# Basant1861/MPC-MMD

Measured on AMD Instinct MI355X. Metric: MPC optimizer steps/s (batch=1024,H=30,obs_samp=500) @1/2/4/8 GPU; % HBM roofline, higher is better.
Workload: dtype f32; 1 GPU; static obs, mmd_opt, batch=1024 rollouts, H=30, num_obs=10, obs_samples=484 (n=22, M=n^2); cost=mmd_opt, global_batch=1024, num_batch=1024, num_prime=30, num_obs=10, num_reduced=22, noise=gaussian, parallelism=config-sharded x1

## Files before the change

### mpc-mmd_amd/csrc/betacem_select.hpp

```cpp
#pragma once
#include "betacem_common.hpp"

namespace mpcmmd {

namespace {

template <int NQ, class V>
DEVI void load_keys(V val, int M, uint32_t* key) {
  const int lane = tidx() & 63;
#pragma unroll
  for (int q = 0; q < NQ; ++q) {
    const int j = lane + 64 * q;
    const float v = val(min(j, M - 1));
    key[q] = j < M ? sort_key_abs(v) : 0u;
  }
}

template <int NQ, int NB>
DEVI void find_thresholds(const uint32_t (*key)[NQ], int nb, int n, uint32_t* T, bool* exact) {
  constexpr int NP = (NB + 1) / 2;
#pragma unroll
  for (int u = 0; u < NB; ++u) {
    T[u] = 0x80000000u;
    exact[u] = u >= nb;
  }
  for (int bit = 30; bit >= 0; --bit) {
    int packed[NP];
#pragma unroll
    for (int i = 0; i < NP; ++i) packed[i] = 0;
#pragma unroll
    for (int u = 0; u < NB; ++u) {
      if (exact[u]) continue;
      const uint32_t cand = T[u] | (1u << bit);
      int c = 0;
#pragma unroll
      for (int q = 0; q < NQ; ++q) c += key[u][q] >= cand;
      packed[u >> 1] += c << (16 * (u & 1));
    }
    bool all = true;
#pragma unroll
    for (int i = 0; i < NP; ++i) {
      const int tot = wave_total(packed[i]);
#pragma unroll
      for (int h = 0; h < 2; ++h) {
        const int u = 2 * i + h;
        if (u >= NB || exact[u]) continue;
        const int cnt = (tot >> (16 * h)) & 0xFFFF;
        if (cnt >= n) T[u] |= 1u << bit;
        exact[u] = cnt == n;
        all = all && exact[u];
      }
    }
    if (all) break;
  }
}

template <int NQ>
DEVI void emit_top(const uint32_t* key, uint32_t T, bool exact, int n, int32_t* out, int* scratch) {
  const int lane = tidx() & 63;
  int need = 0;
  unsigned long long eqm[NQ];
  if (!exact) {
    int gt = 0;
#pragma unroll
    for (int q = 0; q < NQ; ++q) gt += __popcll(__ballot(key[q] > T));
    need = n - gt;
#pragma unroll
    for (int q = 0; q < NQ; ++q) eqm[q] = __ballot(key[q] == T);
  } else {
#pragma unroll
    for (int q = 0; q < NQ; ++q) eqm[q] = 0ull;
  }
  const unsigned long long above = lane == 63 ? 0ull : (~0ull << (lane + 1));
  int* lj = scratch;
  uint32_t* lk = reinterpret_cast<uint32_t*>(scratch + 64);
  int base = 0;
  int later_eq = 0;
#pragma unroll
  for (int q = 0; q < NQ; ++q) later_eq += __popcll(eqm[q]);
#pragma unroll
  for (int q = 0; q < NQ; ++q) {
    later_eq -= __popcll(eqm[q]);
    const int larger = later_eq + __popcll(eqm[q] & above);
    const bool sel = exact ? key[q] >= T : (key[q] > T || (key[q] == T && larger < need));
    const unsigned long long sm = __ballot(sel);
    if (sel) {
      const int pos = base + __popcll(sm & ((1ull << lane) - 1ull));
      lj[pos] = lane + 64 * q;
      lk[pos] = key[q];
    }
    base += __popcll(sm);
  }
  wave_sync();
  const int j = lane < n ? lj[lane] : 0;
  const uint32_t k = lane < n ? lk[lane] : 0xFFFFFFFFu;
  int r = 0;
  for (int c = 0; c < n; ++c) {
    const uint32_t kc = __builtin_amdgcn_readlane(k, c);
    r += (kc < k) || (kc == k && c < lane);
  }
  if (lane < n) out[r] = j;
  wave_sync();
}

template <int NQ, int R>
DEVI bool emit_window(const uint32_t* key, uint32_t T, int n, int32_t* out, unsigned long long* cand) {
  constexpr int cap = 64 * R;
  const int lane = tidx() & 63;
  const unsigned long long below = (1ull << lane) - 1ull;
  int c = 0;
#pragma unroll
  for (int q = 0; q < NQ; ++q) {
    const bool sel = key[q] >= T;
    const unsigned long long m = __ballot(sel);
    const int pos = c + __popcll(m & below);
    cand[sel && pos < cap ? pos : cap + 3] = (static_cast<unsigned long long>(key[q]) << 32) | uint32_t(lane + 64 * q);
    c += __popcll(m);
  }
  if (c > cap) return false;
  if (lane < 8) cand[c + lane] = 0ull;
  wave_sync();
  unsigned long long mine[R];
  int rank[R];
#pragma unroll
  for (int r = 0; r < R; ++r) {
    mine[r] = cand[lane + 64 * r];
    rank[r] = 0;
  }
  const ulonglong2* c2 = reinterpret_cast<const ulonglong2*>(cand);
  for (int e = 0; e < c; e += 8) {
    ulonglong2 v[4];
#pragma unroll
    for (int u = 0; u < 4; ++u) v[u] = c2[(e >> 1) + u];
#pragma unroll
    for (int u = 0; u < 4; ++u)
#pragma unroll
      for (int r = 0; r < R; ++r) rank[r] += int(v[u].x > mine[r]) + int(v[u].y > mine[r]);
  }
#pragma unroll
  for (int r = 0; r < R; ++r)
    if (lane + 64 * r < c && rank[r] < n) out[n - 1 - rank[r]] = int32_t(uint32_t(mine[r]));
  wave_sync();
  return true;
}

template <int CTRL, int ROWS = 0xF>
DEVI uint32_t dpp_umin_src(uint32_t v) {
  return uint32_t(__builtin_amdgcn_update_dpp(-1, int(v), CTRL, ROWS, 0xF, false));
}
DEVI uint32_t wave_min_u32(uint32_t v) {
  v = min(v, dpp_umin_src<0xB1>(v));
  v = min(v, dpp_umin_src<0x4E>(v));
  v = min(v, dpp_umin_src<0x124>(v));
  v = min(v, dpp_umin_src<0x128>(v));
  v = min(v, dpp_umin_src<0x142, 0xA>(v));
  v = min(v, dpp_umin_src<0x143, 0xC>(v));
  return uint32_t(__builtin_amdgcn_readlane(int(v), 63));
}

template <int NQ, int G>
DEVI uint32_t group_max_threshold(const uint32_t* key, int n, uint32_t* lm) {
  const int lane = tidx() & 63;
  uint32_t m = key[0];
#pragma unroll
  for (int q = 1; q < NQ; ++q) m = max(m, key[q]);
  if constexpr (G == 32) m = max(m, uint32_t(__builtin_amdgcn_update_dpp(0, int(m), 0xB1, 0xF, 0xF, false)));
  if (lane % (64 / G) == 0) lm[lane / (64 / G)] = m;
  wave_sync();
  int gt = 0;
  const uint4* l4 = reinterpret_cast<const uint4*>(lm);
#pragma unroll
  for (int e = 0; e < G / 4; ++e) {
    const uint4 v = l4[e];
    gt += int(v.x > m) + int(v.y > m) + int(v.z > m) + int(v.w > m);
  }
  const uint32_t t = wave_min_u32(gt < n ? m : 0xFFFFFFFFu);
  wave_sync();
  return t;
}

template <int NQ, int R, int G, class Row, class Out>
DEVI void select_walk(Row row, Out out, int first, int last, int stride, int M, int n, unsigned long long* cand,
                      uint32_t* lm, int* scratch) {
  uint32_t key[NQ], nxt[NQ];
  load_keys<NQ>(row(first), M, key);
  for (int s = first; s < last; s += stride) {
    load_keys<NQ>(row(min(s + stride, last - 1)), M, nxt);
    bool done = false;
    if (M <= 64 * R)
      done = emit_window<NQ, R>(key, 0x80000000u, n, out(s), cand);
    else if (G > 0 && n <= G * 3 / 4)
      done = emit_window<NQ, R>(key, group_max_threshold<NQ, (G > 0 ? G : 64)>(key, n, lm), n, out(s), cand);
    if (!done) {
      uint32_t Tn[1];
      bool ex[1];
      find_thresholds<NQ, 1>(&key, 1, n, Tn, ex);
      emit_top<NQ>(key, Tn[0], ex[0], n, out(s), scratch);
    }
#pragma unroll
    for (int q = 0; q < NQ; ++q) key[q] = nxt[q];
  }
}

template <int NQ, int R, int G>
DEVI void bselect_wave(const Params& p, int tb, int b, int g, int W, unsigned long long* cand, uint32_t* lm,
                       int* scratch) {
  const int M = p.M, M1 = M + 1, n = p.n;
  int32_t* sel = p.bsel + size_t(b) * kBetaSamples * n;
  float* sig = p.bsig + size_t(b) * kBetaSamples;
  const float* E = p.belite + (size_t(tb & 1) * p.Bt + b) * kBetaElite * M1;
  const int ys = ygen_stride(M);
  const float* Y = p.ygen + size_t(b) * kBzCols * ys;
  const float* z0 = p.beta_z0;
  auto row = [&](int s) {
    const float* r = tb == 0 ? z0 + size_t(s) * M1 : (s < kBetaElite ? E + size_t(s) * M1 : Y + size_t(s - kBetaElite) * ys);
    const bool scale = tb == 0;
    return [=](int j) { return scale ? float(kSqrt20 * double(r[j])) : r[j]; };
  };
  const int s_lo = first_sample(tb);
  if (s_lo + g >= kBetaSamples) return;
  select_walk<NQ, R, G>(row, [&](int s) { return sel + s * n; }, s_lo + g, kBetaSamples, W, M, n, cand, lm, scratch);
  const int lane = tidx() & 63;
  for (int s = s_lo + g + lane * W; lane < 16 && s < kBetaSamples; s += 16 * W) {
    const float v = row(s)(M);
    sig[s] = tb == 0 ? fmaxf(v, 0.01f) : v;
  }
}

}

}
```

### mpc-mmd_amd/csrc/k_bcem_small.hip

```cpp
#define MPCMMD_OPAQUE_TIDX 1
#include "betacem_elite.hpp"
#include "betacem_kernel.hpp"
#include "betacem_qp.hpp"
#include "betacem_sample.hpp"
#include "betacem_select.hpp"

namespace mpcmmd {

namespace {

HDI size_t small_sel_bytes(int R) { return size_t(64 * R + 8) * 8 + 64 * 4 + 128 * 4; }
HDI size_t small_lds(int M, int n, int R, int W) {
  size_t b = size_t(W) * small_sel_bytes(R) + size_t(kNew) * ygen_stride(M) * 4;
  const size_t k = ker_lds(M, n, ker_scratch(M, n, 1, W)).total;
  const size_t d = dir_lds(M, n).total, e = elite_lds(M + 1, W).total;
  const size_t q = (size_t(kBetaSamples) * tri_stride(n) + kQpZeros) * 4;
  const size_t g = size_t(W) * 4 * 32 * 8;
  const size_t gl = ((gen_lds_bytes(M) + 15) & ~size_t(15)) + tblk_lds_bytes(M);
  b = b > q ? b : q;
  b = b > g ? b : g;
  b = b > gl ? b : gl;
  b = b > k ? b : k;
  b = b > d ? b : d;
  b = b > e ? b : e;
  return b;
}

HDI size_t small_persist_off(int M, int n, int R, int W) { return (small_lds(M, n, R, W) + 15) & ~size_t(15); }
HDI size_t small_persist_bytes(int M) { return size_t(M) * (kMomStride + kFeatStride) * 4; }

#define SMALL_STAMP(p, slot)                                                             \
  do {                                                                                   \
    if (tidx() == 0 && (p).dbgw)                                                    \
      (p).dbgw[size_t(32768 + blockIdx.x) * 8 + (slot)] = __builtin_amdgcn_s_memrealtime(); \
  } while (0)

template <int NQ, int R, int G, int NP, int NV4, int GNB, int W>
__global__ __launch_bounds__(64 * W) void k_bcem_small(Params p0, int persist) {
  constexpr int kSmallWaves = W, kSmallThreads = 64 * W;
  extern __shared__ __attribute__((aligned(16))) char smem[];
  const int cand = blockIdx.x;
  const int tid = tidx();
  const int w = __builtin_amdgcn_readfirstlane(tid >> 6);
  const float4* mom_l = nullptr;
  const float4* feat_l = nullptr;
  if (persist) {
    const int M = p0.M, b = p0.b0 + cand;
    float4* pm = reinterpret_cast<float4*>(smem + small_persist_off(M, p0.n, R, W));
    float4* pf = pm + M * (kMomStride / 4);
    const float4* gm = reinterpret_cast<const float4*>(p0.bmom + size_t(b) * M * kMomStride);
    const float4* gf = reinterpret_cast<const float4*>(p0.featr + size_t(b) * M * kFeatStride);
    for (int i = tid; i < M * (kMomStride / 4); i += kSmallThreads) pm[i] = gm[i];
    for (int i = tid; i < M * (kFeatStride / 4); i += kSmallThreads) pf[i] = gf[i];
    mom_l = pm;
    feat_l = pf;
    __syncthreads();
  }
  for (int tb = 0; tb < kBetaIters; ++tb) {
    typedef const Params __attribute__((address_space(4)))* KParams;
    KParams pk = (KParams)__builtin_amdgcn_kernarg_segment_ptr();
    asm volatile("" : "+s"(pk));
    const Params& p = *(const Params*)pk;
    const int b = p.b0 + cand, M = p.M, n = p.n;
    const int ntri = tri_stride(n);
    if (tb > 0) {
      if (tb == 5) SMALL_STAMP(p, 0);
      {
        const int Pp = pos_pad(M);
        const double2* gsrc = reinterpret_cast<const double2*>(p.gen + size_t(b) * Pp * kGenStride);
        const double2* msrc = reinterpret_cast<const double2*>(p.genm + size_t(b) * Pp);
        double2* dst = reinterpret_cast<double2*>(smem);
        const int ng = Pp * kGenRow, nm = Pp >> 1;
        for (int i = tid; i < ng + nm; i += kSmallThreads) dst[i] = i < ng ? gsrc[i] : msrc[i - ng];
        if (tid < 8) dst[ng + nm + tid] = double2{0.0, 0.0};
      }
      __syncthreads();
      {
        const double* lg = reinterpret_cast<const double*>(smem);
        double* Tl = reinterpret_cast<double*>(smem + ((gen_lds_bytes(M) + 15) & ~size_t(15)));
        bsample_tblocks(p, lg, Tl, w, kSmallWaves);
        __syncthreads();
        const int nblk = pos_pad(M) >> 4, units = kSampleTiles * ((nblk + sample_chunk(nblk) - 1) / sample_chunk(nblk));
        for (int u = w; u < units; u += kSmallWaves) bsample_unit_lds(p, tb, b, u % kSampleTiles, u / kSampleTiles, lg, Tl);
      }
      __syncthreads();
      if (tb == 5) SMALL_STAMP(p, 1);
      const int ys = ygen_stride(M);
      const float* Yl = reinterpret_cast<const float*>(smem + size_t(kSmallWaves) * small_sel_bytes(R));
      {
        const float4* src = reinterpret_cast<const float4*>(p.ygen + size_t(b) * kBzCols * ys);
        float4* dst = reinterpret_cast<float4*>(smem + size_t(kSmallWaves) * small_sel_bytes(R));
        for (int i = tid; i < kNew * (ys >> 2); i += kSmallThreads) dst[i] = src[i];
      }
      __syncthreads();
      char* sw = smem + size_t(w) * small_sel_bytes(R);
      unsigned long long* cand_l = reinterpret_cast<unsigned long long*>(sw);
      uint32_t* lm = reinterpret_cast<uint32_t*>(sw + size_t(64 * R + 8) * 8);
      int* scr = reinterpret_cast<int*>(sw + size_t(64 * R + 8) * 8 + 64 * 4);
      {
        int32_t* sel = p.bsel + size_t(b) * kBetaSamples * n;
        float* sig = p.bsig + size_t(b) * kBetaSamples;
        auto row = [&](int s) {
          const float* r = Yl + size_t(s - kBetaElite) * ys;
          return [=](int j) { return r[j]; };
        };
        const int s_lo = first_sample(tb), lane = tid & 63;
        if (s_lo + w < kBetaSamples) {
          select_walk<NQ, R, G>(row, [&](int s) { return sel + s * n; }, s_lo + w, kBetaSamples, kSmallWaves, M, n,
                                cand_l, lm, scr);
          for (int s2 = s_lo + w + lane * kSmallWaves; lane < 16 && s2 < kBetaSamples; s2 += 16 * kSmallWaves)
            sig[s2] = row(s2)(M);
        }
      }
    } else {
      for (int e = tid; e < kBetaSamples * n; e += kSmallThreads) p.bsel[size_t(b) * kBetaSamples * n + e] = p.sel0[e];
      for (int e = tid; e < kBetaSamples; e += kSmallThreads) p.bsig[size_t(b) * kBetaSamples + e] = p.sig0[e];
    }
    __syncthreads();
    if (tb == 5) SMALL_STAMP(p, 2);
    bkernel_body<kSmallWaves, false, true>(p, tb, cand, 0, 1, int(ker_scratch(M, n, tb, kSmallWaves)), smem, mom_l, feat_l);
    __syncthreads();
    if (tb == 5) SMALL_STAMP(p, 3);
    if (tb > 0) {
      const int total = bdirect_total(p, b, 1);
      if (total > 0) {
        bdirect_body<NV4, kSmallWaves>(p, tb, 1, 1, cand, 0, total, smem);
        __syncthreads();
      }
    }
    if (tb == 5) SMALL_STAMP(p, 4);
    {
      const int s_lo = first_sample(tb), per = kBetaSamples - s_lo;
      const float4* src = reinterpret_cast<const float4*>(p.bkred + (size_t(b) * kBetaSamples + s_lo) * ntri);
      float4* kl4 = reinterpret_cast<float4*>(smem);
      for (int i = tid; i < per * (ntri >> 2); i += kSmallThreads) kl4[i] = src[i];
      if (tid < kQpZeros) reinterpret_cast<float*>(smem)[per * ntri + tid] = 0.0f;
      __syncthreads();
      static_assert(kSmallThreads / 4 >= kBetaSamples, "one quad per QP");
      const int g = tid >> 2;
      const bool ok = g < per;
      const int gc = ok ? g : 0;
      bqp_solve<NP>(p, b, s_lo + gc, ok, reinterpret_cast<const float*>(smem) + size_t(gc) * ntri,
                    reinterpret_cast<const float*>(smem) + size_t(per) * ntri);
    }
    __syncthreads();
    if (tb == 5) SMALL_STAMP(p, 5);
    belite_body(p, tb, b, smem);
    __syncthreads();
    if (tb == 5) SMALL_STAMP(p, 6);
    {
      const int nblk = (M + 1 + 15) / 16;
      double* xl = reinterpret_cast<double*>(smem) + 32 * GNB * w;
      for (int blk = w; blk < nblk; blk += kSmallWaves * GNB) bgen_wave<GNB>(p, b, blk, kSmallWaves, xl);
    }
    __syncthreads();
    if (tb == 5) SMALL_STAMP(p, 7);
    if (tb == kBetaIters - 1 && p.bimin[b] >= kBetaElite) {
      bsigma_body(p, tb, b, reinterpret_cast<double*>(smem));
      __syncthreads();
    }
  }
}

}

constexpr int kSmallW512 = 8;
HDI int small_waves(int M) { return M <= 256 ? 16 : (M <= 512 ? kSmallW512 : 8); }

bool bcem_small_ok(const Params& p) {
  return p.gen_wave && p.M <= 256 && p.nb <= 512 && small_lds(p.M, p.n, 1, small_waves(p.M)) <= kLdsBudget;
}

void launch_bcem_small(const Params& p, hipStream_t s) {
  const int n = p.n, M = p.M, W = small_waves(M);
  const dim3 grid(p.nb), block(64 * W);
  const size_t lp = small_persist_off(M, n, 1, W) + small_persist_bytes(M);
  const int persist = lp <= kLdsBudget;
  const size_t lds = persist ? lp : small_lds(M, n, 1, W);
  if (M <= 64)
    hipLaunchKernelGGL((k_bcem_small<1, 1, 32, 8, 1, 1, 16>), grid, block, lds, s, p, persist);
  else if (M <= 128)
    hipLaunchKernelGGL((k_bcem_small<2, 1, 32, 12, 1, 1, 16>), grid, block, lds, s, p, persist);
  else if (M <= 256)
    hipLaunchKernelGGL((k_bcem_small<4, 1, 32, 16, 1, 1, 16>), grid, block, lds, s, p, persist);
  else if (M <= 512)
    hipLaunchKernelGGL((k_bcem_small<8, 1, 32, 24, 2, 16 / kSmallW512, kSmallW512>), grid, block, lds, s,
                       p, persist);
  else
    hipLaunchKernelGGL((k_bcem_small<12, 1, 32, 24, 3, 2, 8>), grid, block, lds, s, p, persist);
}

}
```

### mpc-mmd_amd/csrc/k_bsample.hip

```cpp
#include <algorithm>

#include "betacem_sample.hpp"
#include "betacem_select.hpp"

namespace mpcmmd {

namespace {

__global__ __launch_bounds__(256) void k_bsel0(Params p) {
  const int n = p.n, per = kBetaSamples * n + kBetaSamples;
  for (size_t x = size_t(blockIdx.x) * 256 + tidx(); x < size_t(p.nb) * per; x += size_t(gridDim.x) * 256) {
    const int c = int(x / per), e = int(x - size_t(c) * per), b = p.b0 + c;
    if (e < kBetaSamples * n)
      p.bsel[size_t(b) * kBetaSamples * n + e] = p.sel0[e];
    else
      p.bsig[size_t(b) * kBetaSamples + e - kBetaSamples * n] = p.sig0[e - kBetaSamples * n];
  }
}

template <int TPW>
__global__ __launch_bounds__(64 * sample_waves<TPW>()) void k_bsample(Params p, int tb) {
  const int b = p.b0 + blockIdx.x, M = p.M, Pp = pos_pad(M);
  const int lane = tidx() & 63, w = tidx() >> 6;
  const int r = lane & 15, h = lane >> 4;
  const int s0 = w * TPW * 16;
  MPCMMD_STAMP(p, 0);
  const double* G = p.gen + size_t(b) * Pp * kGenStride;
  const double* gm = p.genm + size_t(b) * Pp;
  const float* z = p.beta_z + size_t(tb - 1) * Pp * kBzCols;
  const int ys = ygen_stride(M);
  float* plane = p.ygen + size_t(b) * kBzCols * ys;
  d4 S[TPW], Sp[TPW], Ya[TPW], Yb[TPW];
#pragma unroll
  for (int t = 0; t < TPW; ++t) {
    S[t] = Sp[t] = d4{0.0, 0.0, 0.0, 0.0};
    Sp[t][2] = h == 3 ? 1.0 : 0.0;
  }
  const int nblk = Pp >> 4, cl = sample_chunk(nblk);
  const __amdgpu_buffer_rsrc_t yr = ygen_rsrc(plane, ys);
  const int vl = (2 * h * ys + r) * 4, v43 = h == 0 ? vl : kDropOffset;
  auto store = [&](const d4* Yv, int q0) {
    if (TPW == kSampleTiles && q0 + 15 < M)
      block_store_rows(Yv, yr, q0, ys, vl, v43);
    else
      block_store<TPW>(Yv, plane, q0, M, ys, s0, r, h);
  };
  SampleBlock<TPW> qa, qb;
  const SampleRsrc srs = sample_rsrc(G, gm, z, Pp, r, h);
  auto load = [&](SampleBlock<TPW>& q, int q0) {
    if constexpr (TPW == kSampleTiles)
      load_block_buf(q, srs, q0);
    else
      load_block(q, G, G + gen_uplane(Pp), gm, z, q0, s0, r, h);
  };
  load(qa, 0);
  for (int c = 0; c < nblk; c += 2) {
    const int p0 = c << 4;
    load(qb, p0 + 16);
    __builtin_amdgcn_sched_barrier(0);
    block_mfma(qa, S, Sp, Ya, r, h);
    __builtin_amdgcn_sched_barrier(0);
    if (c > 0) store(Yb, p0 - 16);
    __builtin_amdgcn_sched_barrier(0);
    load(qa, min(p0 + 32, Pp - 16));
    __builtin_amdgcn_sched_barrier(0);
    block_mfma(qb, S, Sp, Yb, r, h);
    if ((c + 2) % cl == 0)
#pragma unroll
      for (int t = 0; t < TPW; ++t) fold_chunk(Sp[t], S[t]);
    __builtin_amdgcn_sched_barrier(0);
    store(Ya, p0);
    __builtin_amdgcn_sched_barrier(0);
  }
  store(Yb, Pp - 16);
  MPCMMD_STAMP(p, 1);
}

__global__ __launch_bounds__(64 * kChunkWavesMax) void k_bsample_chunks(Params p, int tb) {
  __shared__ double dS[kChunkWavesMax - 1][3][64];
  const int b = p.b0 + blockIdx.x, M = p.M, Pp = pos_pad(M), nblk = Pp >> 4;
  const int lane = tidx() & 63, k = tidx() >> 6, P = blockDim.x >> 6;
  const int r = lane & 15, h = lane >> 4, s0 = blockIdx.y * 16;
  const int cl = sample_chunk(nblk), c0 = k * cl, c1 = min(nblk, c0 + cl);
  MPCMMD_STAMP(p, 0);
  const double* G = p.gen + size_t(b) * Pp * kGenStride;
  const double* gm = p.genm + size_t(b) * Pp;
  const float* z = p.beta_z + size_t(tb - 1) * Pp * kBzCols;
  const int ys = ygen_stride(M);
  float* plane = p.ygen + size_t(b) * kBzCols * ys;
  if (k < P - 1) {
    auto ld = [&](double (&wa)[4], double (&zz)[4], int c) {
#pragma unroll
      for (int kk = 0; kk < 4; ++kk) {
        const size_t pos = size_t(c) * 16 + 4 * kk + h;
        wa[kk] = G[pos * kGenRow + kGenW + r];
        zz[kk] = double(z[bz_index(int(pos), s0 + r)]);
      }
    };
    d4 Sl = d4{0.0, 0.0, 0.0, 0.0};
    double wa[4], zz[4], wn[4], zn[4];
    ld(wa, zz, c0);
    for (int c = c0; c < c1; ++c) {
      ld(wn, zn, min(c + 1, c1 - 1));
#pragma unroll
      for (int kk = 0; kk < 4; ++kk) Sl = mfma64(wa[kk], zz[kk], Sl);
#pragma unroll
      for (int kk = 0; kk < 4; ++kk) {
        wa[kk] = wn[kk];
        zz[kk] = zn[kk];
      }
    }
#pragma unroll
    for (int i = 0; i < 3; ++i) dS[k][i][lane] = Sl[i];
  }
  __syncthreads();
  d4 S[1] = {d4{0.0, 0.0, 0.0, 0.0}}, Sp[1] = {d4{0.0, 0.0, 0.0, 0.0}}, Ya[1], Yb[1];
  Sp[0][2] = h == 3 ? 1.0 : 0.0;
  for (int j = 0; j < k; ++j)
#pragma unroll
    for (int i = 0; i < 3; ++i) Sp[0][i] = Sp[0][i] + dS[j][i][lane];
  SampleBlock<1> qa, qb;
  const int pend = c1 << 4;
  load_block(qa, G, G + gen_uplane(Pp), gm, z, c0 << 4, s0, r, h);
  for (int c = c0; c < c1; c += 2) {
    const int p0 = c << 4;
    load_block(qb, G, G + gen_uplane(Pp), gm, z, p0 + 16, s0, r, h);
    __builtin_amdgcn_sched_barrier(0);
    block_mfma(qa, S, Sp, Ya, r, h);
    __builtin_amdgcn_sched_barrier(0);
    if (c > c0) block_store<1>(Yb, plane, p0 - 16, M, ys, s0, r, h);
    __builtin_amdgcn_sched_barrier(0);
    load_block(qa, G, G + gen_uplane(Pp), gm, z, min(p0 + 32, pend - 16), s0, r, h);
    __builtin_amdgcn_sched_barrier(0);
    block_mfma(qb, S, Sp, Yb, r, h);
    __builtin_amdgcn_sched_barrier(0);
    block_store<1>(Ya, plane, p0, M, ys, s0, r, h);
    __builtin_amdgcn_sched_barrier(0);
  }
  block_store<1>(Yb, plane, pend - 16, M, ys, s0, r, h);
  MPCMMD_STAMP(p, 1);
}

template <int NQ, int R, int G>
__global__ __launch_bounds__(64) void k_bselect(Params p, int tb) {
  __shared__ __attribute__((aligned(16))) unsigned long long cand[64 * R + 8];
  __shared__ __attribute__((aligned(16))) uint32_t lm[64];
  __shared__ int scratch[128];
  if (blockIdx.y == 0 && tidx() == 0) p.bdlcount[size_t(p.b0 + blockIdx.x) * kBetaIters + tb] = 0;
  bselect_wave<NQ, R, G>(p, tb, p.b0 + blockIdx.x, blockIdx.y, gridDim.y, cand, lm, scratch);
}

}

void launch_bsample(const Params& p, int tb, hipStream_t s) {
  if (p.nb >= 384) {
    hipLaunchKernelGGL((k_bsample<6>), dim3(p.nb), dim3(64 * sample_waves<6>()), 0, s, p, tb);
  } else {
    const int nblk = pos_pad(p.M) >> 4, cl = sample_chunk(nblk);
    hipLaunchKernelGGL(k_bsample_chunks, dim3(p.nb, kSampleTiles), dim3(64 * ((nblk + cl - 1) / cl)), 0, s, p, tb);
  }
}

void launch_bsel0(const Params& p, hipStream_t s) {
  const size_t total = size_t(p.nb) * (kBetaSamples * p.n + kBetaSamples);
  hipLaunchKernelGGL(k_bsel0, dim3(unsigned(std::min<size_t>((total + 255) / 256, 4096))), dim3(256), 0, s, p);
}

int sel_waves(int nb, int cap) { return std::max(4, std::min(nb <= 128 ? cap : 16, 16384 / std::max(1, nb))); }

template <int NQ>
void launch_bselect_q(const Params& p, int tb, hipStream_t s) {
  const dim3 grid(p.nb, sel_waves(p.nb, p.sel_cap));
  if (p.n <= 24)
    hipLaunchKernelGGL((k_bselect<NQ, 1, 32>), grid, dim3(64), 0, s, p, tb);
  else if (p.n <= 48)
    hipLaunchKernelGGL((k_bselect<NQ, 2, 64>), grid, dim3(64), 0, s, p, tb);
  else
    hipLaunchKernelGGL((k_bselect<NQ, 2, 0>), grid, dim3(64), 0, s, p, tb);
}

void launch_bselect(const Params& p, int tb, hipStream_t s) {
  const int nq = (p.M + 63) >> 6;
  switch (nq) {
#define MPCMMD_SEL_CASE(q) \
  case q:                  \
    return launch_bselect_q<q>(p, tb, s);
    MPCMMD_SEL_CASE(1)
    MPCMMD_SEL_CASE(2)
    MPCMMD_SEL_CASE(4)
    MPCMMD_SEL_CASE(8)
    MPCMMD_SEL_CASE(16)
#undef MPCMMD_SEL_CASE
    default:
      break;
  }
  if (nq <= 4) return launch_bselect_q<4>(p, tb, s);
  if (nq <= 8) return launch_bselect_q<8>(p, tb, s);
  if (nq <= 12) return launch_bselect_q<12>(p, tb, s);
  if (nq <= 16) return launch_bselect_q<16>(p, tb, s);
  if (nq <= 24) return launch_bselect_q<24>(p, tb, s);
  if (nq <= 32) return launch_bselect_q<32>(p, tb, s);
  if (nq <= 40) return launch_bselect_q<40>(p, tb, s);
  if (nq <= 48) return launch_bselect_q<48>(p, tb, s);
  return launch_bselect_q<64>(p, tb, s);
}

}
```

Measured before the change: 138.2 steps/s.

## Reuse previous top-n threshold and use 32-bit key window selection

Top-n selection now tries a 32-bit key window seeded with a threshold carried over from the previous sample of the same wave. It falls back to the group-max threshold, and then to the 64-bit window or the radix search when the window misses or ties collide. Keys are built with a saturating-add trick, row pointers are made wave-uniform, rows are indexed by byte offset, and the group-max count is split across lane pairs. The kernel also gets a minimum-waves launch bound to raise occupancy. The aim is to skip threshold computation and shrink shared-memory ranking traffic, at the cost of more branches and fallback paths.

```diff
diff --git a/mpc-mmd_amd/csrc/betacem_select.hpp b/mpc-mmd_amd/csrc/betacem_select.hpp
--- a/mpc-mmd_amd/csrc/betacem_select.hpp
+++ b/mpc-mmd_amd/csrc/betacem_select.hpp
@@ -5,15 +5,30 @@
 
 namespace {
 
+DEVI uint32_t select_key(float v) {
+  return __builtin_elementwise_add_sat(__float_as_uint(v) | 0x80000000u, 0x007FFFFEu);
+}
+
 template <int NQ, class V>
 DEVI void load_keys(V val, int M, uint32_t* key) {
-  const int lane = tidx() & 63;
-#pragma unroll
-  for (int q = 0; q < NQ; ++q) {
-    const int j = lane + 64 * q;
-    const float v = val(min(j, M - 1));
-    key[q] = j < M ? sort_key_abs(v) : 0u;
-  }
+  const uint32_t lane = tidx() & 63;
+#pragma unroll
+  for (int q = 0; q < NQ; ++q) {
+    const uint32_t j = lane + 64 * q;
+    const float v = val(4u * min(j, uint32_t(M - 1)));
+    key[q] = j < uint32_t(M) ? select_key(v) : 0u;
+  }
+}
+
+template <class T>
+DEVI T* scalar_ptr(T* p) {
+  const unsigned long long v = reinterpret_cast<unsigned long long>(p);
+  const uint32_t lo = __builtin_amdgcn_readfirstlane(uint32_t(v)), hi = __builtin_amdgcn_readfirstlane(uint32_t(v >> 32));
+  return reinterpret_cast<T*>((static_cast<unsigned long long>(hi) << 32) | lo);
+}
+
+DEVI float row_at(const float* r, uint32_t o) {
+  return *reinterpret_cast<const float*>(reinterpret_cast<const char*>(r) + o);
 }
 
 template <int NQ, int NB>
@@ -104,7 +119,7 @@
 }
 
 template <int NQ, int R>
-DEVI bool emit_window(const uint32_t* key, uint32_t T, int n, int32_t* out, unsigned long long* cand) {
+DEVI bool emit_window64(const uint32_t* key, uint32_t T, int n, int32_t* out, unsigned long long* cand) {
   constexpr int cap = 64 * R;
   const int lane = tidx() & 63;
   const unsigned long long below = (1ull << lane) - 1ull;
@@ -142,6 +157,76 @@
     if (lane + 64 * r < c && rank[r] < n) out[n - 1 - rank[r]] = int32_t(uint32_t(mine[r]));
   wave_sync();
   return true;
+}
+
+enum { kWinMiss = 0, kWinDone = 1, kWinTie = 2 };
+template <int NQ, int R>
+DEVI int emit_window32(const uint32_t* key, uint32_t T, int n, int KR, int32_t* out, uint32_t* ck, uint32_t* lm,
+                       uint32_t& Tc) {
+  constexpr int cap = 64 * R;
+  constexpr bool keep = NQ <= 16;
+  const int lane = tidx() & 63;
+  bool sel[keep ? NQ : 1];
+  unsigned long long msk[keep ? NQ : 1];
+  int c = 0;
+#pragma unroll
+  for (int q = 0; q < NQ; ++q) {
+    const bool s = key[q] >= T;
+    const unsigned long long m = __builtin_amdgcn_ballot_w64(s);
+    if (keep) sel[q] = s, msk[q] = m;
+    c += __popcll(m);
+  }
+  if (c < n || c > cap) return kWinMiss;
+  uint32_t* cj = ck + cap + 8;
+  int base = 0;
+#pragma unroll
+  for (int q = 0; q < NQ; ++q) {
+    const bool s = keep ? sel[q] : key[q] >= T;
+    const unsigned long long m = keep ? msk[q] : __builtin_amdgcn_ballot_w64(s);
+    const int pos = __builtin_amdgcn_mbcnt_hi(uint32_t(m >> 32), __builtin_amdgcn_mbcnt_lo(uint32_t(m), 0u));
+    if (s) {
+      ck[pos + base] = key[q];
+      cj[pos + base] = uint32_t(lane + 64 * q);
+    }
+    base += __popcll(m);
+  }
+  if (lane < 8) ck[c + lane] = 0u;
+  wave_sync();
+  uint32_t mine[R];
+  int rank[R];
+#pragma unroll
+  for (int r = 0; r < R; ++r) {
+    mine[r] = ck[lane + 64 * r];
+    rank[r] = 0;
+  }
+  const uint4* c4 = reinterpret_cast<const uint4*>(ck);
+  for (int e = 0; e < c; e += 8) {
+    const uint4 a = c4[e >> 2], b = c4[(e >> 2) + 1];
+#pragma unroll
+    for (int r = 0; r < R; ++r)
+      rank[r] += int(a.x > mine[r]) + int(a.y > mine[r]) + int(a.z > mine[r]) + int(a.w > mine[r]) +
+                 int(b.x > mine[r]) + int(b.y > mine[r]) + int(b.z > mine[r]) + int(b.w > mine[r]);
+  }
+  bool top[R], clash = false;
+#pragma unroll
+  for (int r = 0; r < R; ++r) {
+    top[r] = lane + 64 * r < c && rank[r] < n;
+    if (top[r]) lm[rank[r]] = uint32_t(lane + 64 * r);
+  }
+  wave_sync();
+#pragma unroll
+  for (int r = 0; r < R; ++r)
+    if (top[r]) clash = clash || lm[rank[r]] != uint32_t(lane + 64 * r);
+  wave_sync();
+  if (__ballot(clash)) return kWinTie;
+  Tc = T;
+#pragma unroll
+  for (int r = 0; r < R; ++r) {
+    if (top[r]) out[n - 1 - rank[r]] = int32_t(cj[lane + 64 * r]);
+    const unsigned long long at = __ballot(lane + 64 * r < c && rank[r] == KR);
+    if (at) Tc = uint32_t(__builtin_amdgcn_readlane(int(mine[r]), __builtin_ctzll(at)));
+  }
+  return kWinDone;
 }
 
 template <int CTRL, int ROWS = 0xF>
@@ -168,12 +253,14 @@
   if (lane % (64 / G) == 0) lm[lane / (64 / G)] = m;
   wave_sync();
   int gt = 0;
-  const uint4* l4 = reinterpret_cast<const uint4*>(lm);
-#pragma unroll
-  for (int e = 0; e < G / 4; ++e) {
+  constexpr int NE = G == 32 ? G / 8 : G / 4;
+  const uint4* l4 = reinterpret_cast<const uint4*>(lm) + (G == 32 ? (lane & 1) * NE : 0);
+#pragma unroll
+  for (int e = 0; e < NE; ++e) {
     const uint4 v = l4[e];
     gt += int(v.x > m) + int(v.y > m) + int(v.z > m) + int(v.w > m);
   }
+  if constexpr (G == 32) gt += __builtin_amdgcn_update_dpp(0, gt, 0xB1, 0xF, 0xF, false);
   const uint32_t t = wave_min_u32(gt < n ? m : 0xFFFFFFFFu);
   wave_sync();
   return t;
@@ -184,13 +271,28 @@
                       uint32_t* lm, int* scratch) {
   uint32_t key[NQ], nxt[NQ];
   load_keys<NQ>(row(first), M, key);
+  constexpr bool can_all = NQ <= R;
+  const bool all = can_all && M <= 64 * R, win = !all && G > 0 && n <= G * 3 / 4;
+  const int KR = all ? 64 * R : n + (n >> 1) - 1;
+  uint32_t* ck = reinterpret_cast<uint32_t*>(cand);
+  uint32_t Tc = 0u;
   for (int s = first; s < last; s += stride) {
     load_keys<NQ>(row(min(s + stride, last - 1)), M, nxt);
     bool done = false;
-    if (M <= 64 * R)
-      done = emit_window<NQ, R>(key, 0x80000000u, n, out(s), cand);
-    else if (G > 0 && n <= G * 3 / 4)
-      done = emit_window<NQ, R>(key, group_max_threshold<NQ, (G > 0 ? G : 64)>(key, n, lm), n, out(s), cand);
+    int step = all ? 2 : (win ? (Tc != 0u ? 0 : 1) : 3);
+    uint32_t T = all ? 0x80000000u : Tc;
+    if constexpr (G > 0 || can_all)
+      while (step < 3) {
+        if constexpr (G > 0)
+          if (step == 1) T = group_max_threshold<NQ, G>(key, n, lm);
+        const int st = emit_window32<NQ, R>(key, T, n, KR, out(s), ck, lm, Tc);
+        if (st == kWinMiss && step == 0) {
+          step = 1;
+          continue;
+        }
+        done = st == kWinDone || (st == kWinTie && emit_window64<NQ, R>(key, T, n, out(s), cand));
+        break;
+      }
     if (!done) {
       uint32_t Tn[1];
       bool ex[1];
@@ -206,27 +308,33 @@
 DEVI void bselect_wave(const Params& p, int tb, int b, int g, int W, unsigned long long* cand, uint32_t* lm,
                        int* scratch) {
   const int M = p.M, M1 = M + 1, n = p.n;
-  int32_t* sel = p.bsel + size_t(b) * kBetaSamples * n;
+  int32_t* sel = scalar_ptr(p.bsel + size_t(b) * kBetaSamples * n);
   float* sig = p.bsig + size_t(b) * kBetaSamples;
-  const float* E = p.belite + (size_t(tb & 1) * p.Bt + b) * kBetaElite * M1;
   const int ys = ygen_stride(M);
-  const float* Y = p.ygen + size_t(b) * kBzCols * ys;
+  const float* Y = scalar_ptr(p.ygen + size_t(b) * kBzCols * ys);
   const float* z0 = p.beta_z0;
-  auto row = [&](int s) {
-    const float* r = tb == 0 ? z0 + size_t(s) * M1 : (s < kBetaElite ? E + size_t(s) * M1 : Y + size_t(s - kBetaElite) * ys);
-    const bool scale = tb == 0;
-    return [=](int j) { return scale ? float(kSqrt20 * double(r[j])) : r[j]; };
-  };
   const int s_lo = first_sample(tb);
   if (s_lo + g >= kBetaSamples) return;
-  select_walk<NQ, R, G>(row, [&](int s) { return sel + s * n; }, s_lo + g, kBetaSamples, W, M, n, cand, lm, scratch);
-  const int lane = tidx() & 63;
-  for (int s = s_lo + g + lane * W; lane < 16 && s < kBetaSamples; s += 16 * W) {
-    const float v = row(s)(M);
-    sig[s] = tb == 0 ? fmaxf(v, 0.01f) : v;
-  }
-}
-
-}
-
-}
+  const int lane = tidx() & 63;
+  auto run = [&](auto row, bool clip) {
+    select_walk<NQ, R, G>(row, [&](int s) { return sel + s * n; }, s_lo + g, kBetaSamples, W, M, n, cand, lm, scratch);
+    for (int s = s_lo + g + lane * W; lane < 16 && s < kBetaSamples; s += 16 * W) {
+      const float v = row(s)(4u * M);
+      sig[s] = clip ? fmaxf(v, 0.01f) : v;
+    }
+  };
+  if (tb == 0)
+    run([&](int s) {
+      const float* r = z0 + size_t(s) * M1;
+      return [=](uint32_t o) { return float(kSqrt20 * double(row_at(r, o))); };
+    }, true);
+  else
+    run([&](int s) {
+      const float* r = Y + size_t(s - kBetaElite) * ys;
+      return [=](uint32_t o) { return row_at(r, o); };
+    }, false);
+}
+
+}
+
+}
diff --git a/mpc-mmd_amd/csrc/k_bcem_small.hip b/mpc-mmd_amd/csrc/k_bcem_small.hip
--- a/mpc-mmd_amd/csrc/k_bcem_small.hip
+++ b/mpc-mmd_amd/csrc/k_bcem_small.hip
@@ -102,14 +102,14 @@
         float* sig = p.bsig + size_t(b) * kBetaSamples;
         auto row = [&](int s) {
           const float* r = Yl + size_t(s - kBetaElite) * ys;
-          return [=](int j) { return r[j]; };
+          return [=](uint32_t o) { return row_at(r, o); };
         };
         const int s_lo = first_sample(tb), lane = tid & 63;
         if (s_lo + w < kBetaSamples) {
           select_walk<NQ, R, G>(row, [&](int s) { return sel + s * n; }, s_lo + w, kBetaSamples, kSmallWaves, M, n,
                                 cand_l, lm, scr);
           for (int s2 = s_lo + w + lane * kSmallWaves; lane < 16 && s2 < kBetaSamples; s2 += 16 * kSmallWaves)
-            sig[s2] = row(s2)(M);
+            sig[s2] = row(s2)(4u * M);
         }
       }
     } else {
diff --git a/mpc-mmd_amd/csrc/k_bsample.hip b/mpc-mmd_amd/csrc/k_bsample.hip
--- a/mpc-mmd_amd/csrc/k_bsample.hip
+++ b/mpc-mmd_amd/csrc/k_bsample.hip
@@ -141,8 +141,12 @@
   MPCMMD_STAMP(p, 1);
 }
 
+constexpr int select_min_waves(int NQ, int R) {
+  return NQ <= 4 ? 8 : NQ <= 8 ? (R == 1 ? 6 : 5) : NQ <= 16 ? 4 : NQ <= 24 ? 3 : NQ <= 32 ? 2 : 1;
+}
+
 template <int NQ, int R, int G>
-__global__ __launch_bounds__(64) void k_bselect(Params p, int tb) {
+__global__ __launch_bounds__(64, select_min_waves(NQ, R)) void k_bselect(Params p, int tb) {
   __shared__ __attribute__((aligned(16))) unsigned long long cand[64 * R + 8];
   __shared__ __attribute__((aligned(16))) uint32_t lm[64];
   __shared__ int scratch[128];
```

Result: no change. 139.1 steps/s, median of 6 (+0.7%).
